# meyer-lab/cmtf-pls

Hardware: AMD Instinct MI355X
Metric: nipals_iters_per_sec (higher is better)
Workload: dtype f32

## Files before the change

cmtf_pls_amd/_lib.py:

```python
from __future__ import annotations

import ctypes
import os
from ctypes import c_char_p, c_double, c_int, c_int64, c_size_t, c_uint32, c_uint64, c_void_p

_HERE = os.path.dirname(os.path.abspath(__file__))
LIB_PATH = os.environ.get("CMTFPLS_LIB") or os.path.join(_HERE, "lib", "libcmtfpls.so")

_P = c_void_p

class XcovBlock(ctypes.Structure):
    _fields_ = [("S", _P), ("S2", _P), ("colcnt", _P), ("n_samples", c_double), ("order", c_int), ("A", c_int), ("B", c_int),
                ("n_squarings", c_int), ("Z", _P), ("wA", _P), ("wB", _P), ("info", _P)]


class KfoldState(ctypes.Structure):
    _fields_ = [("I", c_int), ("A", c_int), ("B", c_int), ("M", c_int), ("K", c_int), ("R", c_int)] + [
        (name, _P) for name in ("fold_of", "S", "mean", "Yk", "Gy", "WA", "WB", "Q", "Wa", "Wb", "T", "Gt", "coef", "Rm", "tm",
                                "Tout", "vec", "n_iter", "status", "part")]


class CvCoupledBlock(ctypes.Structure):
    _fields_ = [("X", _P), ("order", c_int), ("A", c_int), ("B", c_int)]


class LooCoupledBlock(ctypes.Structure):
    _fields_ = [("X", _P), ("colsum", _P), ("order", c_int), ("A", c_int), ("B", c_int)]


SIGNATURES = {
    "cmtfpls_xcov_iterate_blocks_f64": (c_int, [ctypes.POINTER(XcovBlock), c_int, c_int, _P, _P, _P, _P, _P, c_int, _P, c_size_t, _P]),
    "cmtfpls_abi_version": (c_int, []),
    "cmtfpls_last_error": (c_char_p, []),
    "cmtfpls_clear_error": (c_int, []),
    "cmtfpls_status_to_host": (c_int, [_P, _P, c_size_t, _P, _P]),
    "cmtfpls_colstats_workspace_bytes": (c_size_t, [c_int64, c_int64]),
    "cmtfpls_colstats_f32": (c_int, [_P, c_int64, c_int64, _P, _P, _P, c_size_t, _P]),
    "cmtfpls_colstats_f64": (c_int, [_P, c_int64, c_int64, _P, _P, _P, c_size_t, _P]),
    "cmtfpls_sweep_partials": (c_int, []),
    "cmtfpls_center_f32": (c_int, [_P, c_int64, c_int64, _P, _P, _P, _P]),
    "cmtfpls_center_f64": (c_int, [_P, c_int64, c_int64, _P, _P, _P, _P]),
    "cmtfpls_mode0_contract_workspace_bytes": (c_size_t, [c_int64, c_int64]),
# ... 115 lines not shown
                                          _P, _P, c_size_t, _P]),
    "cmtfpls_heldout_resid_f64": (c_int, [_P, c_int64, c_int, c_int, _P, c_int, c_int, _P, _P, _P, c_double, c_uint64, c_uint32, c_uint64,
                                          _P, _P, c_size_t, _P]),
    "cmtfpls_impute_workspace_bytes": (c_size_t, [c_int64, c_int64]),
    "cmtfpls_impute_f32": (c_int, [_P, _P, c_int64, c_int, c_int, _P, c_int, c_int, _P, _P, _P, _P, _P, c_size_t, _P]),
    "cmtfpls_impute_f64": (c_int, [_P, _P, c_int64, c_int, c_int, _P, c_int, c_int, _P, _P, _P, _P, _P, c_size_t, _P]),
    "cmtfpls_loo_fold_workspace_bytes": (c_size_t, [c_int, c_int, c_int, c_int, c_int]),
    "cmtfpls_loo_tpls_f64": (c_int, [_P, _P, _P, _P, c_int, c_int, c_int, c_int, c_int, c_double, c_int, c_int, c_int, _P, _P, _P, c_size_t, _P]),
    "cmtfpls_loo_xcov_fold_workspace_bytes": (c_size_t, [c_int, c_int, c_int, c_int, c_int]),
    "cmtfpls_kfold_xcov_workspace_bytes": (c_size_t, [c_int64, c_int64, c_int, c_int]),
    "cmtfpls_kfold_xcov_f32": (c_int, [_P, c_int64, c_int, c_int, _P, c_int, _P, _P, c_int, _P, _P, _P, _P, _P, c_size_t, _P]),
    "cmtfpls_kfold_xcov_f64": (c_int, [_P, c_int64, c_int, c_int, _P, c_int, _P, _P, c_int, _P, _P, _P, _P, _P, c_size_t, _P]),
    "cmtfpls_kfold_xcov_bf16": (c_int, [_P, c_int64, c_int, c_int, _P, c_int, _P, _P, c_int, _P, _P, _P, _P, _P, c_size_t, _P]),
    "cmtfpls_kfold_xcov_f16": (c_int, [_P, c_int64, c_int, c_int, _P, c_int, _P, _P, c_int, _P, _P, _P, _P, _P, c_size_t, _P]),
    "cmtfpls_kfold_row_tiles": (c_int, [c_int64]),
    "cmtfpls_kfold_part_stride": (c_int, []),
    "cmtfpls_kfold_inner_workspace_bytes": (c_size_t, [c_int, c_int, c_int]),
    "cmtfpls_kfold_inner_f64": (c_int, [ctypes.POINTER(KfoldState), c_int, c_double, c_int, _P, c_size_t, _P]),
    "cmtfpls_kfold_inner_tensor_workspace_bytes": (c_size_t, [c_int, c_int, c_int, c_int]),
    "cmtfpls_kfold_inner_tensor_lds_bytes": (c_size_t, [c_int, c_int, c_int, c_int]),
    "cmtfpls_kfold_inner_tensor_f64": (c_int, [ctypes.POINTER(KfoldState), _P, c_int, c_int, c_int, c_int, c_double, c_int, _P, _P, _P,
                                       c_size_t, _P]),
    "cmtfpls_kfold_epilogue_f64": (c_int, [ctypes.POINTER(KfoldState), c_int, c_int, _P, _P]),
    "cmtfpls_kfold_inner_coupled_workspace_bytes": (c_size_t, [ctypes.POINTER(KfoldState), c_int]),
    "cmtfpls_kfold_inner_coupled_f64": (c_int, [ctypes.POINTER(KfoldState), c_int, c_int, c_double, c_int, _P, c_size_t, _P]),
    "cmtfpls_kfold_inner_coupled_tensor_workspace_bytes": (c_size_t, [ctypes.POINTER(KfoldState), c_int, ctypes.POINTER(c_int)]),
    "cmtfpls_kfold_inner_coupled_tensor_lds_bytes": (c_size_t, [ctypes.POINTER(KfoldState), c_int, ctypes.POINTER(c_int)]),
    "cmtfpls_kfold_inner_coupled_tensor_f64": (c_int, [ctypes.POINTER(KfoldState), c_int, ctypes.POINTER(c_int), _P, c_int, c_int, c_double,
                                                       c_int, _P, _P, _P, c_size_t, _P]),
    "cmtfpls_kfold_combine_scores_f64": (c_int, [_P, c_int, c_int64, _P, _P]),
    "cmtfpls_kfold_wide_xcov_workspace_bytes": (c_size_t, [c_int64, c_int64, c_int, c_int]),
    "cmtfpls_kfold_wide_xcov_f32": (c_int, [_P, c_int64, c_int, c_int, _P, c_int, _P, _P, c_int, _P, _P, _P, _P, _P, c_size_t, _P]),
    "cmtfpls_kfold_wide_xcov_f64": (c_int, [_P, c_int64, c_int, c_int, _P, c_int, _P, _P, c_int, _P, _P, _P, _P, _P, c_size_t, _P]),
    "cmtfpls_kfold_wide_xcov_bf16": (c_int, [_P, c_int64, c_int, c_int, _P, c_int, _P, _P, c_int, _P, _P, _P, _P, _P, c_size_t, _P]),
    "cmtfpls_kfold_wide_xcov_f16": (c_int, [_P, c_int64, c_int, c_int, _P, c_int, _P, _P, c_int, _P, _P, _P, _P, _P, c_size_t, _P]),
    "cmtfpls_kfold_inner_grouped_f64": (c_int, [ctypes.POINTER(KfoldState), _P, c_int, c_int, c_double, c_int, _P, c_size_t, _P]),
    "cmtfpls_kfold_inner_coupled_grouped_f64": (c_int, [ctypes.POINTER(KfoldState), c_int, _P, c_int, c_int, c_double, c_int, _P, c_size_t,
                                                        _P]),
    "cmtfpls_kfold_epilogue_grouped_f64": (c_int, [ctypes.POINTER(KfoldState), _P, c_int, c_int, c_int, _P, _P]),
    "cmtfpls_kfold_epilogue_splits_f64": (c_int, [ctypes.POINTER(KfoldState), c_int, c_int, c_int, _P, _P]),
    "cmtfpls_kfold_weighted_xcov_workspace_bytes": (c_size_t, [c_int64, c_int64, c_int, c_int]),
    "cmtfpls_kfold_weighted_xcov_f32": (c_int, [_P, c_int64, c_int, c_int, _P, c_int, c_int, _P, _P, _P, _P, c_size_t, _P]),
    "cmtfpls_kfold_weighted_xcov_f64": (c_int, [_P, c_int64, c_int, c_int, _P, c_int, c_int, _P, _P, _P, _P, c_size_t, _P]),
    "cmtfpls_kfold_weighted_xcov_bf16": (c_int, [_P, c_int64, c_int, c_int, _P, c_int, c_int, _P, _P, _P, _P, c_size_t, _P]),
    "cmtfpls_kfold_weighted_xcov_f16": (c_int, [_P, c_int64, c_int, c_int, _P, c_int, c_int, _P, _P, _P, _P, c_size_t, _P]),
    "cmtfpls_kfold_epilogue_weighted_f64": (c_int, [ctypes.POINTER(KfoldState), c_int, c_int, _P, _P]),
# ... 78 lines not shown
```

cmtf_pls_amd/backend.py:

```python
from __future__ import annotations

import ctypes
from typing import Optional, Tuple

import torch

from . import _lib
from .storage import HALF_DTYPES, HALF_ENTRIES, SUFFIX, entry_name

_HALF_ENTRIES = tuple(dict.fromkeys(e for group in HALF_ENTRIES.values() for e in group))


def _ptr(t: Optional[torch.Tensor]):
    return None if t is None else t.data_ptr()


def _int_pairs(pairs):
    flat = [int(v) for p in pairs for v in p]
    return (ctypes.c_int * len(flat))(*flat)


def _scratch(nbytes: int, device) -> torch.Tensor:
    return torch.empty(max(int(nbytes), 256), dtype=torch.uint8, device=device)

# ... 304 lines not shown
        keep = (blocks, q_cur, tq, q_new, G, status, wr, arr)
        fn, stream = self.lib.cmtfpls_xcov_iterate_blocks_f64, self._stream
        args = (nb, M, _ptr(q_cur), _ptr(tq), _ptr(q_new), _ptr(G), status[0:1].data_ptr())
        tail = (_ptr(wr), wr.numel())

        def enqueue(n_squarings, first: bool, _keep=keep) -> None:
            for i in range(nb):
                arr[i].n_squarings = int(n_squarings[i])
            rc = fn(arr, *args, 1 if first else 0, *tail, stream())
            if rc:
                _lib.check(rc, "xcov_iterate_blocks")
        return enqueue

    def s_downdate(self, S: torch.Tensor, A: int, B: int, ya: torch.Tensor, wA: torch.Tensor, wB: torch.Tensor,
                   q: torch.Tensor, v: torch.Tensor) -> None:
        assert S.is_contiguous() and S.shape[1] == A * B
        _lib.check(self.lib.cmtfpls_s_downdate_f64(_ptr(S), S.shape[0], A, B, _ptr(ya), _ptr(wA), _ptr(wB), _ptr(q), _ptr(v),
                                                   self._stream()), "s_downdate")

    def kr_axpy(self, v: torch.Tensor, A: int, B: int, WA: torch.Tensor, WB: torch.Tensor, k: int, coef: torch.Tensor) -> torch.Tensor:
        assert WA.is_contiguous() and WB.is_contiguous() and WA.shape[1] == WB.shape[1] and coef.numel() >= k
        _lib.check(self.lib.cmtfpls_kr_axpy_f64(_ptr(v), A, B, _ptr(WA), _ptr(WB), WA.shape[1], int(k), _ptr(coef), self._stream()), "kr_axpy")
        return v

    def axpy_scalar(self, y: torch.Tensor, a: torch.Tensor, x: Optional[torch.Tensor] = None) -> torch.Tensor:
        assert y.is_contiguous() and y.dtype == torch.float64 and a.numel() >= 1 and (x is None or (x.is_contiguous() and x.numel() == y.numel()))
        _lib.check(self.lib.cmtfpls_axpy_scalar_f64(_ptr(y), y.numel(), _ptr(a), _ptr(x), self._stream()), "axpy_scalar")
        return y

    def total(self, v: torch.Tensor) -> torch.Tensor:
        assert v.is_contiguous() and v.dtype == torch.float64
        return self._close_partials(v)

    def quadform(self, G: torch.Tensor, q: torch.Tensor, q_old: torch.Tensor, out: torch.Tensor) -> torch.Tensor:
        _lib.check(self.lib.cmtfpls_quadform_f64(_ptr(G), G.shape[0], _ptr(q), _ptr(q_old), _ptr(out), self._stream()), "quadform")
        return out

    def mttkrp(self, X2: torch.Tensor, A: int, B: int, WA: torch.Tensor, WB: torch.Tensor, out: torch.Tensor,
               mixed: bool = False) -> Optional[torch.Tensor]:
        R = WA.shape[1]
        assert WA.is_contiguous() and WB.is_contiguous() and out.stride(1) == 1
        fn = self._read_fn("mttkrp", X2, mixed)
        if fn is None:
            return None
        rc = fn(_ptr(X2), X2.shape[0], A, B, _ptr(WA), _ptr(WB), R, _ptr(out), out.stride(0), self._stream())
        return self._form(rc, "mttkrp", out)
# ... 608 lines not shown
```

cmtf_pls_amd/csrc/solve.hip:

```cpp
#include "common.hpp"

namespace cmtfpls {

constexpr int kSolveMax = 64;

__global__ __launch_bounds__(kSolveMax) void normal_solve_kernel(const double* __restrict__ G, const double* __restrict__ g, int k,
                                                                double* __restrict__ b, int incb) {
  __shared__ double A[kSolveMax][kSolveMax + 1];
  __shared__ double d[kSolveMax], y[kSolveMax];
  __shared__ int dep[kSolveMax];
  const int i = threadIdx.x;
  if (i < k) {
    const double gii = G[(int64_t)i * k + i];
    d[i] = (gii > 0.0 && isfinite(gii)) ? 1.0 / sqrt(gii) : 0.0;
    dep[i] = 0;
  }
  __syncthreads();
  if (i < k) {
    for (int j = 0; j < k; ++j) A[i][j] = G[(int64_t)i * k + j] * d[i] * d[j];
    y[i] = g[i] * d[i];
  }
  __syncthreads();
  const double tiny = (double)k * 2.220446049250313e-16;
  for (int c = 0; c < k; ++c) {
    const double piv = A[c][c];
    const bool ok = piv > tiny;
    __syncthreads();
    if (ok) {
      const double l = sqrt(piv);
      if (i == c) A[c][c] = l;
      if (i > c && i < k) A[i][c] = A[i][c] / l;
    } else {
      if (i == c) { A[c][c] = 1.0; dep[c] = 1; }
      if (i > c && i < k) A[i][c] = 0.0;
    }
    __syncthreads();
    if (ok && i > c && i < k) {
      const double lic = A[i][c];
      for (int j = c + 1; j <= i; ++j) A[i][j] -= lic * A[j][c];
    }
    __syncthreads();
  }
  if (i == 0) {
    for (int r = 0; r < k; ++r) {
      double s = y[r];
      for (int j = 0; j < r; ++j) s -= A[r][j] * y[j];
      y[r] = dep[r] ? 0.0 : s / A[r][r];
    }
    for (int r = k - 1; r >= 0; --r) {
      double s = y[r];
      for (int j = r + 1; j < k; ++j) s -= A[j][r] * y[j];
      y[r] = dep[r] ? 0.0 : s / A[r][r];
    }
  }
  __syncthreads();
  if (i < k) b[(int64_t)i * incb] = y[i] * d[i];
}

constexpr int kSolveBigMax = 1024;
__global__ __launch_bounds__(256) void normal_solve_big_kernel(const double* __restrict__ G, const double* __restrict__ g, int k,
                                                               double* __restrict__ b, int incb, double* __restrict__ Aw) {
  const int ld = k + 1;
  double* d = Aw + (size_t)k * ld;
  double* y = d + k;
  double* depf = y + k;
  __shared__ double s_piv;
  const int t = threadIdx.x;
  for (int i = t; i < k; i += 256) {
    const double gii = G[(int64_t)i * k + i];
    d[i] = (gii > 0.0 && isfinite(gii)) ? 1.0 / sqrt(gii) : 0.0;
    depf[i] = 0.0;
  }
  __syncthreads();
  for (int i = t; i < k; i += 256) {
    for (int j = 0; j < k; ++j) Aw[(size_t)i * ld + j] = G[(int64_t)i * k + j] * d[i] * d[j];
    y[i] = g[i] * d[i];
  }
  __syncthreads();
  const double tiny = (double)k * 2.220446049250313e-16;
// ... 181 lines not shown
```

cmtf_pls_amd/fitrun.py:

```python
from __future__ import annotations

import math
from typing import Dict, List, Optional

import numpy as np
import torch

from .fitrun_xcov import XcovMixin
from .sparsity import SWITCHED_OFF, resolve_sparsity, validate_sparse_limits
from .state import BlockState, FitState, split_trailing, validate_limits
from .storage import HALF_DTYPES, HALF_ENTRIES, dtype_name, fallback_text, half_route


class FitRun(XcovMixin):

    def __init__(self, eng: NipalsEngine, Xs: List[torch.Tensor], Y: torch.Tensor, n_components: int, coupled: bool,
                 algorithm: str = "direct", owned: Optional[List[bool]] = None, allow_raw: bool = True, sparsity=None):
        be, comm = eng.be, eng.comm
        Xs = list(Xs)
        owned = [True] * len(Xs) if owned is None else list(owned)
        if algorithm not in ("direct", "xcov"):
            raise ValueError("algorithm must be 'direct' or 'xcov'")
        self.algorithm_requested = self.algorithm = algorithm
        self.notes: List[str] = []
# ... 258 lines not shown
            if self.S12[b] is not None:
                self.Yw[:, :self.M].copy_(self.Y)
                torch.mul(self.Y, self.rowscale[b][:, None], out=self.Yw[:, self.M:])
                be.xcov(self.X2[b], self.Yw, True, out=self.S12[b], mixed=self.mixed)
                comm.allreduce(self.S12[b])
                continue
            if b in self._s_prebuilt:
                del self._s_prebuilt[b]
            elif self.raw and self._ssq_with_s and b not in self._ssq0_dev:
                _, ssq = be.xcov_ssq(self.X2[b], self.Y, blk.mean, out=self.S[b])
                self._ssq0_dev[b] = comm.allreduce(ssq)
            else:
                be.xcov(self.X2[b], self.Y, blk.has_miss, out=self.S[b], mixed=self.mixed)
            comm.allreduce(self.S[b])
            if self.raw:
                ysum, _ = be.colstats(self.Y)
                comm.allreduce(ysum)
                be.s_downdate(self.S[b], blk.A, blk.B, self.zM, self.zA[b], self.zB[b], ysum, blk.mean)
            if blk.has_miss:
                torch.mul(self.Y, self.rowscale[b][:, None], out=self.Yw)
                be.xcov(self.X2[b], self.Yw, True, out=self.S2[b], mixed=self.mixed)
                comm.allreduce(self.S2[b])
        self._s_ready = False
        be.gram_tn(self.Y, self.Y, out=self.Gy)
        comm.allreduce(self.Gy)
        self._parity = 0
        self.qc = self.qx[0]
        self.qc.zero_()
        self.qc[0] = 1.0

    def inner_loop(self, a: int, max_iter: int, tol: float, verbose: int = 0) -> None:
        if max_iter > 0 and self._pipeline_ok():
            self._pipelined = True
            self._inner_loop_xcov_pipelined(a, max_iter, tol, verbose)
            return
        for it in range(max_iter):
            du = self.iterate(it)
            if du is not None and du < tol:
                if verbose:
                    print("Comp {}: converged after {} iterations".format(a, it))
                break

    def _sparse_arg(self, b: int):
        if self.sparse is None:
            return None
        return self.sparse[b], (self.sparse_info[b] if len(self.blocks[b].shape) == 3 else None)

    def _sparse_count(self, b: int) -> None:
        if self.sparse is None or len(self.blocks[b].shape) != 3:
            return
        acc, inf = self.sparse_acc[b], self.sparse_info[b]
        acc[0:1].add_(1.0 - inf[0:1])
# ... 431 lines not shown
            rep["x_copy"] = "centred private copy"
        else:
            nowrite = bool(getattr(self, "_nowrite", False))
            one_read = nowrite and bool(getattr(self, "_one_read", False))
            any_miss = any(b.has_miss for b in self.blocks)
            rep["x_copy"] = "none: the caller's uncentred tensor is read in place" if self.raw else "centred private copy"
            rep["raw"] = bool(self.raw)
            rep["x_written"] = not nowrite
            rep["s_carried"] = bool(self._s_carry)
            rep["s_build"] = ("per component (missing values)" if any_miss else "first component only") + \
                             (f", {(self.M + 63) // 64} response tiles of <= 64" if self.M > 64 else "") + \
                             (", [Y, Y * rowscale] in one pass" if any(x is not None for x in self.S12) else "")
            rep["one_read"] = one_read
            rep["stats_with_s"] = bool(getattr(self, "_stats_with_s", False))
            if nowrite:
                rep["x_passes_per_component"] = ("1 read (largest block); 2 reads (other blocks)" if one_read and nb > 1 else
                                                 "1 read" if one_read else "2 reads")
            elif any_miss and nb == 1 and getattr(self, "_deflate_build_ok", True) and self.S12[0] is not None and eng.opt.xcov_deflate_build:
                rep["x_passes_per_component"] = "1 read + 1 read + write (deflation inside the rebuild of S)"
            elif any_miss:
                rep["x_passes_per_component"] = "1 read + write (score + deflation) + S rebuild reads"
            else:
                rep["x_passes_per_component"] = "1 read + 1 read + write"
            rep["pipelined"] = bool(getattr(self, "_pipelined", False))
            if rep["pipelined"]:
                rep["pipeline"] = dict(self.pipeline_stats)
            if not rep["pipelined"] and eng.opt.xcov_pipeline:
                why = ("sparse loadings" if self.sparse is not None else "graph replay requested" if self.use_graphs else "more than 64 responses" if self.M > 64 else
                       "a block of order > 3 or a backend without the single-call iteration")
                self.notes.append("inner loop on S not pipelined: " + why)
            if self.algorithm_requested == "xcov" and not self.raw and eng.opt.xcov_raw and not any_miss and not any("uncentred" in n for n in self.notes):
                self.notes.append("uncentred xcov form declined: " + ("more than 64 components" if self.R > 64 else
                                                                      "f32 matrix precision or a backend without its kernels"))
            if nowrite and eng.opt.xcov_one_read and self.R > 1 and not one_read:
                self.notes.append("one read per component declined: the row does not fit the registers of 1..16 workgroups "
                                  "(rows of 2048..131072 f32 -- 262144 when the last mode divides 4096 -- / 1024..131072 f64 elements, "
                                  "last mode a multiple of 4 / 2)")
        if any(d is not None for d in self.half_storage):
            rep["half_storage"] = {
                "in_place": self.half_fallback is None,
                "fallback": self.half_fallback,
                "reads": [None if d is None or self.half_fallback is not None else self._half_reads_form(b)
                          for b, d in enumerate(self.half_storage)],
            }
        rep["rank1_one_launch_chain"] = bool(getattr(eng.be, "rank1_chain_side", 0)) and any(
            len(blk.shape) == 3 and min(blk.A, blk.B) <= int(getattr(eng.be, "rank1_chain_side", 0)) for blk in self.blocks)
# ... 30 lines not shown
```

cmtf_pls_amd/fitrun_xcov.py:

```python
from __future__ import annotations

import math
from typing import Optional

import torch

from .storage import HALF_DTYPES


class XcovMixin:
    def _score_x0(self, b: int, out: torch.Tensor) -> None:
        be, blk, X2 = self.eng.be, self.blocks[b], self.X2[b]
        if X2.dtype in HALF_DTYPES:
            self.half_reads.setdefault(b, set()).add("mttkrp")
            if be.mttkrp(X2, blk.A, blk.B, self.wA[b].view(-1, 1), self.wB[b].view(-1, 1), out.view(-1, 1)) is None:
                raise RuntimeError("mttkrp refused a shape the 16-bit fit was planned for")
        else:
            be.score(X2, blk.A, blk.B, self.wA[b], self.wB[b], None, out)

    def _contract_x0(self, b: int, v: torch.Tensor, out: torch.Tensor) -> None:
        be, X2 = self.eng.be, self.X2[b]
        if X2.dtype in HALF_DTYPES:
            self.half_reads.setdefault(b, set()).add("xcov")
            if be.xcov(X2, v.view(-1, 1), False, out=out.view(1, -1)) is None:
# ... 236 lines not shown
                if a > 0:
                    be.rowdot(self.T[:, :a], g, self.corr, None)
                    corr = self.corr
                if nb == 2:
                    others = self.Ts[1 - b]
                elif nb > 2:
                    others = self.Ts[[x for x in range(nb) if x != b]].sum(dim=0)
                one_read = be.score_contract(self.X2[b], blk.A, blk.B, self.wA[b], self.wB[b], mw, self.Ts[b], self.ps,
                                             sub_own=corr, add_other=others, alpha=1.0 / nb,
                                             csum=self.csum if self.raw else None) is not None
                if one_read:
                    if self.X2[b].dtype in HALF_DTYPES:
                        self.half_reads.setdefault(b, set()).add("score_contract")
                    continue
                self._one_read = False
            self._score_x0(b, self.Ts[b])
            if mw is not None:
                be.axpy_scalar(self.Ts[b], mw)
            if a > 0:
                be.y_deflate(self.Ts[b].view(I, 1), self.T, a, g, self.one)
        single = self.t.data_ptr() == self.Ts.data_ptr()
        if not single:
            be.scores_mean(self.Ts, self.t)
        if one_read:
            comm.allreduce(self.ps)
            if self.raw:
                be.axpy_scalar(self.ps, comm.allreduce(self.csum), self.blocks[fused_b].mean)
            self.Rm[:, a].copy_(self.ps)
        be.rowdot(self.Y, self.q, self.u, None)
        be.gram_tn(self.t, self.t, out=self.dot_log[a, 0:1])
        for b in range(nb):
            if single:
                self.dot_log[a, 1 + b].copy_(self.dot_log[a, 0])
            else:
                be.gram_tn(self.Ts[b], self.t, out=self.dot_log[a, 1 + b: 2 + b])
        self.T[:, a].copy_(self.t)
        self.U[:, a].copy_(self.u)
        self.Q[:, a].copy_(self.q)
        Ta = self.T[:, :k]
        ya = be.gram_tn(self.Y, self.t).reshape(-1)
        b_dev, ya_g = self._inner_regression(a, extra=ya)
        if k < R and not (one_read and nb == 1):
            be.rowdot(Ta, b_dev, self.yhat.view(-1), None)
        ssqy = be.y_deflate(self.Y, self.T, k, b_dev, self.q)
        if k < R:
            c = be.gram_tn(self._G_last, b_dev).reshape(-1)
            for b, blk in enumerate(self.blocks):
                WA, WB = self.eng._kr_operands(blk, R)
                if one_read and b == fused_b:
                    be.rowdot(self.Rm[:, :k], b_dev, self.vs[b], None)
                else:
                    self._contract_x0(b, self.yhat.view(-1), self.vs[b])
                    comm.allreduce(self.vs[b])
                    if self.raw:
                        be.axpy_scalar(self.vs[b], comm.allreduce(be.total(self.yhat.view(-1))), blk.mean)
                be.kr_axpy(self.vs[b], blk.A, blk.B, WA, WB, k, c)
                be.s_downdate(self.S[b], blk.A, blk.B, ya_g, self.wA[b], self.wB[b], self.q, self.vs[b])
            self._s_ready = True
        self.ssq_log[a, nb].copy_(ssqy.reshape(()))
```

cmtf_pls_amd/options.py:

```python
from __future__ import annotations

from dataclasses import dataclass, replace
from typing import Optional


@dataclass(frozen=True)
class EngineOptions:
    small_fit: bool = True
    small_fit_elements: int = 1 << 15
    xcov_nowrite: bool = True
    xcov_raw: bool = True
    xcov_raw_max_offset: float = 1e4
    project_raw_max_offset: float = 1e4
    xcov_one_read: bool = True
    xcov_pair_build: bool = True
    xcov_ssq_with_s: bool = True
    xcov_stats_with_s: bool = True
    xcov_deflate_build: bool = True
    xcov_pipeline: bool = True
    capture_collectives: bool = False
    project_split_rows: bool = True
    masked_folds: bool = False
    masked_folds_coupled: bool = False
    coupled_permutations: bool = False
    tensor_folds: bool = False
    tensor_folds_coupled: bool = False
    masked_tensor_folds: bool = False
    tensor_resamples_coupled: bool = False
    masked_tensor_folds_coupled: bool = False
    half_folds: bool = False
    half_diagnostics: bool = False
    sparse_tol: float = 1e-10
    sparse_max_sweeps: int = 200

    def but(self, **changes) -> "EngineOptions":
        return replace(self, **changes)

# ... 13 lines not shown
```

include/cmtfpls.h:

```cpp
#ifndef CMTFPLS_H
#define CMTFPLS_H

#include <stddef.h>
#include <stdint.h>

#ifdef __cplusplus
extern "C" {
#endif

#define CMTFPLS_OK 0
#define CMTFPLS_EINVAL 1
#define CMTFPLS_EWORKSPACE 2
#define CMTFPLS_EHIP 3
#define CMTFPLS_EUNSUPPORTED 4

int cmtfpls_abi_version(void);
const char* cmtfpls_last_error(void);
int cmtfpls_clear_error(void);
int cmtfpls_status_to_host(const void* src, void* dst_host, size_t bytes, void* event, void* stream);

size_t cmtfpls_colstats_workspace_bytes(int64_t I, int64_t P);
int cmtfpls_colstats_f32(const float* X, int64_t I, int64_t P, double* colsum, double* colcnt,
                         void* ws, size_t ws_bytes, void* stream);
int cmtfpls_colstats_f64(const double* X, int64_t I, int64_t P, double* colsum, double* colcnt,
// ... 397 lines not shown
int cmtfpls_kfold_inner_coupled_grouped_f64(const cmtfpls_kfold_state* blocks, int nb, const int* model_fold, int groups, int a, double tol,
                                            int max_iter, void* ws, size_t ws_bytes, void* stream);

int cmtfpls_kfold_epilogue_splits_f64(const cmtfpls_kfold_state* st, int splits, int stage, int a, const double* in, void* stream);

size_t cmtfpls_kfold_weighted_xcov_workspace_bytes(int64_t I, int64_t P, int n, int M);
int cmtfpls_kfold_weighted_xcov_f32(const float* X, int64_t I, int A, int B, const double* Y, int n, int M, double* S, double* mean,
                                    double* stats, void* ws, size_t ws_bytes, void* stream);
int cmtfpls_kfold_weighted_xcov_f64(const double* X, int64_t I, int A, int B, const double* Y, int n, int M, double* S, double* mean,
                                    double* stats, void* ws, size_t ws_bytes, void* stream);
int cmtfpls_kfold_weighted_xcov_bf16(const uint16_t* X, int64_t I, int A, int B, const double* Y, int n, int M, double* S, double* mean,
                                     double* stats, void* ws, size_t ws_bytes, void* stream);
int cmtfpls_kfold_weighted_xcov_f16(const uint16_t* X, int64_t I, int A, int B, const double* Y, int n, int M, double* S, double* mean,
                                    double* stats, void* ws, size_t ws_bytes, void* stream);
int cmtfpls_kfold_epilogue_weighted_f64(const cmtfpls_kfold_state* st, int stage, int a, const double* in, void* stream);
size_t cmtfpls_press_rows_workspace_bytes(int n, int64_t I, int R, int M);
int cmtfpls_press_rows_f64(const double* T, const double* coef, const double* Q, const double* nu, const double* Y, const int* eval,
                           int n, int64_t I, int R, int M, double* press, double* pred, void* ws, size_t ws_bytes, void* stream);
size_t cmtfpls_fit_small_workspace_bytes(int I, int A, int B, int M);
int cmtfpls_fit_small_f64(const double* X, const double* Y, int I, int A, int B, int M, int R, double tol, int max_iter,
                          double* T, double* U, double* WA, double* WB, double* Q, double* coef, double* ssq, double* x_mean,
                          double* y_mean, int* n_iter, int* flag, void* ws, size_t ws_bytes, void* stream);

int cmtfpls_add_noise_f32(float* X, int64_t n, double sigma, uint64_t seed, uint64_t offset, double nan_fraction,
                          void* stream);
int cmtfpls_add_noise_f64(double* X, int64_t n, double sigma, uint64_t seed, uint64_t offset, double nan_fraction,
                          void* stream);

int cmtfpls_ceiling_max_blocks(void);
int cmtfpls_ceiling_read(const void* buf, size_t bytes, int64_t row_bytes, int map, float* sink, int blocks, void* stream);
int cmtfpls_ceiling_rmw(void* buf, size_t bytes, int64_t row_bytes, int map, int blocks, void* stream);
int cmtfpls_ceiling_copy(const void* src, void* dst, size_t bytes, int64_t row_bytes, int map, int blocks, void* stream);

#ifdef __cplusplus
}
#endif
#endif
```

Measured before the change: 764.6.

## Fuse per-component NIPALS boundary steps into five tiled device launches

Adds a device entry that does the end-of-component work (score/U store, T'T and T'U reductions, normal-equation solve, Y deflation with Gy rebuild, S downdate, q reset) in five kernels. Before, this was a long sequence of separate small launches and host-driven steps. The fit path now calls it for single order-3 blocks and skips the Gy recompute and q reset afterwards. The intent is to cut launch count and host overhead at component boundaries, at the cost of a large new code path with fixed tiling and shape limits.

Result: no change. 763.9 (-0.1%).

```diff
diff --git a/cmtf_pls_amd/_lib.py b/cmtf_pls_amd/_lib.py
--- a/cmtf_pls_amd/_lib.py
+++ b/cmtf_pls_amd/_lib.py
@@ -18,6 +18,12 @@
     _fields_ = [("I", c_int), ("A", c_int), ("B", c_int), ("M", c_int), ("K", c_int), ("R", c_int)] + [
         (name, _P) for name in ("fold_of", "S", "mean", "Yk", "Gy", "WA", "WB", "Q", "Wa", "Wb", "T", "Gt", "coef", "Rm", "tm",
                                 "Tout", "vec", "n_iter", "status", "part")]
+
+
+class XcovBoundaryArgs(ctypes.Structure):
+    _fields_ = [("I", c_int64)] + [(name, c_int) for name in ("M", "R", "a", "A", "B", "raw")] + [
+        (name, _P) for name in ("t", "Y", "q", "T", "U", "G", "b", "coef", "c", "ya", "dots", "Q", "wA", "wB", "LA", "LB", "q_next",
+                                "Gy", "ssq", "S", "ps", "csum", "mean", "Rm")]
 
 
 class CvCoupledBlock(ctypes.Structure):
@@ -179,6 +185,9 @@
     "cmtfpls_kfold_inner_tensor_f64": (c_int, [ctypes.POINTER(KfoldState), _P, c_int, c_int, c_int, c_int, c_double, c_int, _P, _P, _P,
                                        c_size_t, _P]),
     "cmtfpls_kfold_epilogue_f64": (c_int, [ctypes.POINTER(KfoldState), c_int, c_int, _P, _P]),
+    "cmtfpls_xcov_boundary_tiles": (c_int, []),
+    "cmtfpls_xcov_boundary_workspace_bytes": (c_size_t, [c_int64, c_int, c_int, c_int64]),
+    "cmtfpls_xcov_boundary_f64": (c_int, [ctypes.POINTER(XcovBoundaryArgs), c_int, _P, c_size_t, _P]),
     "cmtfpls_kfold_inner_coupled_workspace_bytes": (c_size_t, [ctypes.POINTER(KfoldState), c_int]),
     "cmtfpls_kfold_inner_coupled_f64": (c_int, [ctypes.POINTER(KfoldState), c_int, c_int, c_double, c_int, _P, c_size_t, _P]),
     "cmtfpls_kfold_inner_coupled_tensor_workspace_bytes": (c_size_t, [ctypes.POINTER(KfoldState), c_int, ctypes.POINTER(c_int)]),
diff --git a/cmtf_pls_amd/backend.py b/cmtf_pls_amd/backend.py
--- a/cmtf_pls_amd/backend.py
+++ b/cmtf_pls_amd/backend.py
@@ -350,6 +350,24 @@
         assert WA.is_contiguous() and WB.is_contiguous() and WA.shape[1] == WB.shape[1] and coef.numel() >= k
         _lib.check(self.lib.cmtfpls_kr_axpy_f64(_ptr(v), A, B, _ptr(WA), _ptr(WB), WA.shape[1], int(k), _ptr(coef), self._stream()), "kr_axpy")
         return v
+
+    def xcov_boundary_args(self, **fields):
+        args = _lib.XcovBoundaryArgs()
+        for name, value in fields.items():
+            self.xcov_boundary_set(args, name, value)
+        return args
+
+    @staticmethod
+    def xcov_boundary_set(args, name: str, value) -> None:
+        if isinstance(value, torch.Tensor):
+            assert value.dtype == torch.float64 and value.is_contiguous(), name
+            value = value.data_ptr()
+        setattr(args, name, value)
+
+    def xcov_boundary(self, args, stage: int = 0) -> Optional[bool]:
+        ws = self._workspace("xcov_boundary", self.lib.cmtfpls_xcov_boundary_workspace_bytes(args.I, args.M, args.R, args.A * args.B))
+        rc = self.lib.cmtfpls_xcov_boundary_f64(ctypes.byref(args), int(stage), _ptr(ws), ws.numel(), self._stream())
+        return self._form(rc, "xcov_boundary")
 
     def axpy_scalar(self, y: torch.Tensor, a: torch.Tensor, x: Optional[torch.Tensor] = None) -> torch.Tensor:
         assert y.is_contiguous() and y.dtype == torch.float64 and a.numel() >= 1 and (x is None or (x.is_contiguous() and x.numel() == y.numel()))
diff --git a/cmtf_pls_amd/csrc/boundary.hip b/cmtf_pls_amd/csrc/boundary.hip
--- /dev/null
+++ b/cmtf_pls_amd/csrc/boundary.hip
@@ -0,0 +1,312 @@
+#include "common.hpp"
+#include "normal_solve.hpp"
+
+namespace cmtfpls {
+
+constexpr int kBndTiles = 256;
+constexpr int kBndMaxM = 64, kBndMaxR = 64;
+constexpr int kBndStage = 4096;
+
+__device__ __forceinline__ void bnd_reduce16(const double (&acc)[16], int n, double (*red)[16], double* out) {
+  const int lane = threadIdx.x & 63, wv = threadIdx.x >> 6;
+#pragma unroll
+  for (int e = 0; e < 16; ++e) {
+    const double w = wave_sum(acc[e]);
+    if (lane == 0) red[wv][e] = w;
+  }
+  __syncthreads();
+  if ((int)threadIdx.x < n) {
+    const int e = threadIdx.x;
+    out[e] = ((red[0][e] + red[1][e]) + red[2][e]) + red[3][e];
+  }
+  __syncthreads();
+}
+
+__global__ __launch_bounds__(256) void boundary_rows_kernel(cmtfpls_xcov_boundary_args p, double* __restrict__ part) {
+  __shared__ double red[4][16];
+  __shared__ double qs[kBndMaxM];
+  const int tid = threadIdx.x;
+  const int M = p.M, R = p.R, a = p.a, k = a + 1;
+  const int64_t I = p.I;
+  for (int m = tid; m < M; m += 256) qs[m] = p.q[m];
+  __syncthreads();
+  const int64_t first = (int64_t)blockIdx.x * 256 + tid, step = (int64_t)kBndTiles * 256;
+  double* out = part + (int64_t)blockIdx.x * (2 * R + M);
+  if (M <= 16) {
+    double acc[16];
+#pragma unroll
+    for (int e = 0; e < 16; ++e) acc[e] = 0.0;
+    for (int64_t i = first; i < I; i += step) {
+      const double ti = p.t[i];
+      const double* yr = p.Y + i * M;
+      double s = 0.0;
+#pragma unroll
+      for (int e = 0; e < 16; ++e)
+        if (e < M) {
+          const double y = yr[e];
+          s = fma(y, qs[e], s);
+          acc[e] = fma(y, ti, acc[e]);
+        }
+      p.U[i * R + a] = s;
+      p.T[i * R + a] = ti;
+    }
+    bnd_reduce16(acc, M, red, out + 2 * R);
+  } else {
+    for (int64_t i = first; i < I; i += step) {
+      const double* yr = p.Y + i * M;
+      double s = 0.0;
+      for (int m = 0; m < M; ++m) s = fma(yr[m], qs[m], s);
+      p.U[i * R + a] = s;
+      p.T[i * R + a] = p.t[i];
+    }
+  }
+  __syncthreads();
+  for (int m0 = 0; m0 < M && M > 16; m0 += 16) {
+    const int mc = (M - m0 < 16) ? M - m0 : 16;
+    double acc[16];
+#pragma unroll
+    for (int e = 0; e < 16; ++e) acc[e] = 0.0;
+    for (int64_t i = first; i < I; i += step) {
+      const double ti = p.t[i];
+      const double* yr = p.Y + i * M + m0;
+#pragma unroll
+      for (int e = 0; e < 16; ++e)
+        if (e < mc) acc[e] = fma(yr[e], ti, acc[e]);
+    }
+    bnd_reduce16(acc, mc, red, out + 2 * R + m0);
+  }
+  for (int j0 = 0; j0 < k; j0 += 16) {
+    const int jc = (k - j0 < 16) ? k - j0 : 16;
+    double at[16], au[16];
+#pragma unroll
+    for (int e = 0; e < 16; ++e) { at[e] = 0.0; au[e] = 0.0; }
+    for (int64_t i = first; i < I; i += step) {
+      const double ti = p.t[i], ui = p.U[i * R + a];
+      const double* tr = p.T + i * R + j0;
+#pragma unroll
+      for (int e = 0; e < 16; ++e)
+        if (e < jc) {
+          const double tv = tr[e];
+          at[e] = fma(tv, ti, at[e]);
+          au[e] = fma(tv, ui, au[e]);
+        }
+    }
+    bnd_reduce16(at, jc, red, out + j0);
+    bnd_reduce16(au, jc, red, out + R + j0);
+  }
+}
+
+__global__ __launch_bounds__(256) void boundary_solve_kernel(cmtfpls_xcov_boundary_args p, const double* __restrict__ part) {
+  __shared__ NormalSolveLds s;
+  __shared__ double tt[kBndMaxR], tu[kBndMaxR], bs[kBndMaxR];
+  const int tid = threadIdx.x;
+  const int M = p.M, R = p.R, a = p.a, k = a + 1, stride = 2 * R + M;
+  const int lane = tid & 63, wv = tid >> 6;
+  for (int o = wv; o < 2 * k + M; o += 4) {
+    const int col = (o < k) ? o : (o < 2 * k) ? R + (o - k) : 2 * R + (o - 2 * k);
+    double v = 0.0;
+    for (int tile = lane; tile < kBndTiles; tile += 64) v += part[(int64_t)tile * stride + col];
+    v = wave_sum(v);
+    if (lane == 0) {
+      if (o < k) tt[o] = v;
+      else if (o < 2 * k) tu[o - k] = v;
+      else p.ya[o - 2 * k] = v;
+    }
+  }
+  __syncthreads();
+  if (tid < k) {
+    p.G[(int64_t)a * R + tid] = tt[tid];
+    p.G[(int64_t)tid * R + a] = tt[tid];
+  }
+  if (tid == 0) { p.dots[0] = tt[a]; p.dots[1] = tt[a]; }
+  __syncthreads();
+  const double bi = normal_solve_block(p.G, R, tu, k, s);
+  if (tid < k) {
+    bs[tid] = bi;
+    p.b[tid] = bi;
+    p.coef[(int64_t)tid * R + a] = bi;
+  }
+  __syncthreads();
+  if (tid < k) {
+    double v = 0.0;
+    for (int j = 0; j < k; ++j) v = fma(p.G[(int64_t)tid * R + j], bs[j], v);
+    p.c[tid] = v;
+  }
+  for (int m = tid; m < M; m += 256) p.Q[(int64_t)m * R + a] = p.q[m];
+  for (int i = tid; i < p.A; i += 256) p.LA[(int64_t)i * R + a] = p.wA[i];
+  for (int i = tid; i < p.B; i += 256) p.LB[(int64_t)i * R + a] = p.wB[i];
+}
+
+__global__ __launch_bounds__(256) void boundary_ydefl_kernel(cmtfpls_xcov_boundary_args p, double* __restrict__ part) {
+  __shared__ double Ys[kBndStage];
+  __shared__ double qs[kBndMaxM], bs[kBndMaxR], red[16];
+  const int tid = threadIdx.x;
+  const int M = p.M, R = p.R, k = p.a + 1, MM = M * M, TR = (kBndStage / M < 256) ? kBndStage / M : 256;
+  for (int m = tid; m < M; m += 256) qs[m] = p.q[m];
+  for (int j = tid; j < k; j += 256) bs[j] = p.b[j];
+  __syncthreads();
+  const int64_t rows_per = (p.I + kBndTiles - 1) / kBndTiles;
+  const int64_t r0 = (int64_t)blockIdx.x * rows_per;
+  const int64_t r1 = (r0 + rows_per < p.I) ? r0 + rows_per : p.I;
+  double ssq = 0.0;
+  double acc[16];
+#pragma unroll
+  for (int e = 0; e < 16; ++e) acc[e] = 0.0;
+  for (int64_t rb = r0; rb < r1; rb += TR) {
+    const int nr = (int)((r1 - rb < TR) ? r1 - rb : TR);
+    if (tid < nr) {
+      const int64_t i = rb + tid;
+      double yh = 0.0;
+      for (int j = 0; j < k; ++j) yh = fma(p.T[i * R + j], bs[j], yh);
+      double* yr = p.Y + i * M;
+      for (int m = 0; m < M; ++m) {
+        const double v = yr[m] - yh * qs[m];
+        yr[m] = v;
+        Ys[tid * M + m] = v;
+        ssq = fma(v, v, ssq);
+      }
+    }
+    __syncthreads();
+#pragma unroll
+    for (int e = 0; e < 16; ++e) {
+      const int o = tid + e * 256;
+      if (o < MM) {
+        const int m1 = o / M, m2 = o % M;
+        double v = acc[e];
+        for (int r = 0; r < nr; ++r) v = fma(Ys[r * M + m1], Ys[r * M + m2], v);
+        acc[e] = v;
+      }
+    }
+    __syncthreads();
+  }
+  double* out = part + (int64_t)blockIdx.x * (MM + 1);
+#pragma unroll
+  for (int e = 0; e < 16; ++e) {
+    const int o = tid + e * 256;
+    if (o < MM) out[o] = acc[e];
+  }
+  const double tot = block_sum(ssq, red);
+  if (tid == 0) out[MM] = tot;
+}
+
+__global__ __launch_bounds__(256) void boundary_close_kernel(cmtfpls_xcov_boundary_args p, const double* __restrict__ part) {
+  const int M = p.M, MM = M * M;
+  const int o = blockIdx.x * 4 + (threadIdx.x >> 6), lane = threadIdx.x & 63;
+  if (o <= MM) {
+    double v = 0.0;
+    for (int tile = lane; tile < kBndTiles; tile += 64) v += part[(int64_t)tile * (MM + 1) + o];
+    v = wave_sum(v);
+    if (lane == 0) {
+      if (o < MM) p.Gy[o] = v;
+      else p.ssq[0] = v;
+    }
+  }
+  if (blockIdx.x == 0 && p.q_next && (int)threadIdx.x < M) p.q_next[threadIdx.x] = threadIdx.x == 0 ? 1.0 : 0.0;
+}
+
+__global__ __launch_bounds__(256) void boundary_downdate_kernel(cmtfpls_xcov_boundary_args p) {
+  __shared__ double bs[kBndMaxR], cs[kBndMaxR], yas[kBndMaxM], qs[kBndMaxM];
+  const int tid = threadIdx.x;
+  const int M = p.M, R = p.R, a = p.a, k = a + 1, B = p.B;
+  for (int j = tid; j < k; j += 256) { bs[j] = p.b[j]; cs[j] = p.c[j]; }
+  for (int m = tid; m < M; m += 256) { yas[m] = p.ya[m]; qs[m] = p.q[m]; }
+  __syncthreads();
+  const int64_t P = (int64_t)p.A * B;
+  const int64_t c = (int64_t)blockIdx.x * 256 + tid;
+  if (c >= P) return;
+  const int64_t ia = c / B, ib = c % B;
+  double r = p.ps[c];
+  if (p.raw) r = fma(-p.csum[0], p.mean[c], r);
+  double* rm = p.Rm + c * R;
+  rm[a] = r;
+  double v = 0.0;
+  for (int j = 0; j < a; ++j) v = fma(rm[j], bs[j], v);
+  v = fma(r, bs[a], v);
+  const double* wa = p.LA + ia * R;
+  const double* wb = p.LB + ib * R;
+  double w2 = 0.0;
+  for (int j = 0; j < k; ++j) w2 = fma(cs[j] * wa[j], wb[j], w2);
+  v -= w2;
+  const double w = p.wA[ia] * p.wB[ib];
+  for (int m = 0; m < M; ++m) {
+    double sv = p.S[(int64_t)m * P + c];
+    sv = fma(-yas[m], w, sv);
+    sv = fma(-qs[m], v, sv);
+    p.S[(int64_t)m * P + c] = sv;
+  }
+}
+
+static size_t bnd_part1(int M, int R) { return (size_t)kBndTiles * (size_t)(2 * R + M); }
+static size_t bnd_part3(int M) { return (size_t)kBndTiles * (size_t)(M * M + 1); }
+
+}
+
+using namespace cmtfpls;
+
+extern "C" {
+
+int cmtfpls_xcov_boundary_tiles(void) { return kBndTiles; }
+
+size_t cmtfpls_xcov_boundary_workspace_bytes(int64_t I, int M, int R, int64_t P) {
+  (void)I;
+  (void)P;
+  if (M <= 0 || R <= 0 || M > kBndMaxM || R > kBndMaxR) return 0;
+  return (bnd_part1(M, R) + bnd_part3(M)) * sizeof(double);
+}
+
+int cmtfpls_xcov_boundary_f64(const cmtfpls_xcov_boundary_args* p, int stage, void* ws, size_t ws_bytes, void* stream) {
+  if (!p || stage < 0 || stage > 5) { set_error("xcov_boundary: bad argument"); return CMTFPLS_EINVAL; }
+  if (p->I <= 0 || p->M <= 0 || p->R <= 0 || p->A <= 0 || p->B <= 0 || p->a < 0 || p->a >= p->R) {
+    set_error("xcov_boundary: bad argument");
+    return CMTFPLS_EINVAL;
+  }
+  if (p->M > kBndMaxM || p->R > kBndMaxR || p->I > ((int64_t)1 << 38) || (int64_t)p->A * p->B > ((int64_t)1 << 38)) {
+    set_error("xcov_boundary: shape outside the device form (M <= 64, R <= 64); use the separate entries");
+    return CMTFPLS_EUNSUPPORTED;
+  }
+  const bool last = p->a + 1 >= p->R;
+  const bool all = stage == 0;
+  const bool s1 = all || stage == 1, s2 = all || stage == 2, s3 = all || stage == 3, s4 = all || stage == 4;
+  const bool s5 = (all && !last) || stage == 5;
+  if (((s1 || s2 || s3 || s5) && !p->q) || (s1 && (!p->t || !p->Y || !p->T || !p->U)) ||
+      (s2 && (!p->G || !p->b || !p->coef || !p->c || !p->ya || !p->dots || !p->Q || !p->wA || !p->wB || !p->LA || !p->LB)) ||
+      (s3 && (!p->Y || !p->T || !p->b)) || (s4 && (!p->Gy || !p->ssq)) ||
+      (s5 && (!p->S || !p->ps || !p->Rm || !p->b || !p->c || !p->ya || !p->wA || !p->wB || !p->LA || !p->LB ||
+              (p->raw && (!p->csum || !p->mean))))) {
+    set_error("xcov_boundary: bad argument");
+    return CMTFPLS_EINVAL;
+  }
+  if (!ws || ws_bytes < cmtfpls_xcov_boundary_workspace_bytes(p->I, p->M, p->R, (int64_t)p->A * p->B)) {
+    set_error("xcov_boundary: workspace too small");
+    return CMTFPLS_EWORKSPACE;
+  }
+  hipStream_t st = (hipStream_t)stream;
+  double* part1 = static_cast<double*>(ws);
+  double* part3 = part1 + bnd_part1(p->M, p->R);
+  const int MM1 = p->M * p->M + 1;
+  const int64_t P = (int64_t)p->A * p->B;
+  int rc = CMTFPLS_OK;
+  if (s1) {
+    hipLaunchKernelGGL(boundary_rows_kernel, dim3(kBndTiles), dim3(256), 0, st, *p, part1);
+    rc = check_launch("xcov_boundary: rows");
+  }
+  if (rc == CMTFPLS_OK && s2) {
+    hipLaunchKernelGGL(boundary_solve_kernel, dim3(1), dim3(256), 0, st, *p, part1);
+    rc = check_launch("xcov_boundary: solve");
+  }
+  if (rc == CMTFPLS_OK && s3) {
+    hipLaunchKernelGGL(boundary_ydefl_kernel, dim3(kBndTiles), dim3(256), 0, st, *p, part3);
+    rc = check_launch("xcov_boundary: ydefl");
+  }
+  if (rc == CMTFPLS_OK && s5) {
+    hipLaunchKernelGGL(boundary_downdate_kernel, dim3((unsigned)((P + 255) / 256)), dim3(256), 0, st, *p);
+    rc = check_launch("xcov_boundary: downdate");
+  }
+  if (rc == CMTFPLS_OK && s4) {
+    hipLaunchKernelGGL(boundary_close_kernel, dim3((unsigned)((MM1 + 3) / 4)), dim3(256), 0, st, *p, part3);
+    rc = check_launch("xcov_boundary: close");
+  }
+  return rc;
+}
+
+}
diff --git a/cmtf_pls_amd/csrc/normal_solve.hpp b/cmtf_pls_amd/csrc/normal_solve.hpp
--- /dev/null
+++ b/cmtf_pls_amd/csrc/normal_solve.hpp
@@ -0,0 +1,63 @@
+#pragma once
+#include "common.hpp"
+
+namespace cmtfpls {
+
+constexpr int kSolveMax = 64;
+
+struct NormalSolveLds {
+  double A[kSolveMax][kSolveMax + 1];
+  double d[kSolveMax], y[kSolveMax];
+  int dep[kSolveMax];
+};
+
+__device__ __forceinline__ double normal_solve_block(const double* G, int ldg, const double* g, int k, NormalSolveLds& s) {
+  const int i = threadIdx.x;
+  if (i < k) {
+    const double gii = G[(int64_t)i * ldg + i];
+    s.d[i] = (gii > 0.0 && isfinite(gii)) ? 1.0 / sqrt(gii) : 0.0;
+    s.dep[i] = 0;
+  }
+  __syncthreads();
+  if (i < k) {
+    for (int j = 0; j < k; ++j) s.A[i][j] = G[(int64_t)i * ldg + j] * s.d[i] * s.d[j];
+    s.y[i] = g[i] * s.d[i];
+  }
+  __syncthreads();
+  const double tiny = (double)k * 2.220446049250313e-16;
+  for (int c = 0; c < k; ++c) {
+    const double piv = s.A[c][c];
+    const bool ok = piv > tiny;
+    __syncthreads();
+    if (ok) {
+      const double l = sqrt(piv);
+      if (i == c) s.A[c][c] = l;
+      if (i > c && i < k) s.A[i][c] = s.A[i][c] / l;
+    } else {
+      if (i == c) { s.A[c][c] = 1.0; s.dep[c] = 1; }
+      if (i > c && i < k) s.A[i][c] = 0.0;
+    }
+    __syncthreads();
+    if (ok && i > c && i < k) {
+      const double lic = s.A[i][c];
+      for (int j = c + 1; j <= i; ++j) s.A[i][j] -= lic * s.A[j][c];
+    }
+    __syncthreads();
+  }
+  if (i == 0) {
+    for (int r = 0; r < k; ++r) {
+      double v = s.y[r];
+      for (int j = 0; j < r; ++j) v -= s.A[r][j] * s.y[j];
+      s.y[r] = s.dep[r] ? 0.0 : v / s.A[r][r];
+    }
+    for (int r = k - 1; r >= 0; --r) {
+      double v = s.y[r];
+      for (int j = r + 1; j < k; ++j) v -= s.A[j][r] * s.y[j];
+      s.y[r] = s.dep[r] ? 0.0 : v / s.A[r][r];
+    }
+  }
+  __syncthreads();
+  return i < k ? s.y[i] * s.d[i] : 0.0;
+}
+
+}
diff --git a/cmtf_pls_amd/csrc/solve.hip b/cmtf_pls_amd/csrc/solve.hip
--- a/cmtf_pls_amd/csrc/solve.hip
+++ b/cmtf_pls_amd/csrc/solve.hip
@@ -1,60 +1,13 @@
 #include "common.hpp"
+#include "normal_solve.hpp"
 
 namespace cmtfpls {
-
-constexpr int kSolveMax = 64;
 
 __global__ __launch_bounds__(kSolveMax) void normal_solve_kernel(const double* __restrict__ G, const double* __restrict__ g, int k,
                                                                 double* __restrict__ b, int incb) {
-  __shared__ double A[kSolveMax][kSolveMax + 1];
-  __shared__ double d[kSolveMax], y[kSolveMax];
-  __shared__ int dep[kSolveMax];
-  const int i = threadIdx.x;
-  if (i < k) {
-    const double gii = G[(int64_t)i * k + i];
-    d[i] = (gii > 0.0 && isfinite(gii)) ? 1.0 / sqrt(gii) : 0.0;
-    dep[i] = 0;
-  }
-  __syncthreads();
-  if (i < k) {
-    for (int j = 0; j < k; ++j) A[i][j] = G[(int64_t)i * k + j] * d[i] * d[j];
-    y[i] = g[i] * d[i];
-  }
-  __syncthreads();
-  const double tiny = (double)k * 2.220446049250313e-16;
-  for (int c = 0; c < k; ++c) {
-    const double piv = A[c][c];
-    const bool ok = piv > tiny;
-    __syncthreads();
-    if (ok) {
-      const double l = sqrt(piv);
-      if (i == c) A[c][c] = l;
-      if (i > c && i < k) A[i][c] = A[i][c] / l;
-    } else {
-      if (i == c) { A[c][c] = 1.0; dep[c] = 1; }
-      if (i > c && i < k) A[i][c] = 0.0;
-    }
-    __syncthreads();
-    if (ok && i > c && i < k) {
-      const double lic = A[i][c];
-      for (int j = c + 1; j <= i; ++j) A[i][j] -= lic * A[j][c];
-    }
-    __syncthreads();
-  }
-  if (i == 0) {
-    for (int r = 0; r < k; ++r) {
-      double s = y[r];
-      for (int j = 0; j < r; ++j) s -= A[r][j] * y[j];
-      y[r] = dep[r] ? 0.0 : s / A[r][r];
-    }
-    for (int r = k - 1; r >= 0; --r) {
-      double s = y[r];
-      for (int j = r + 1; j < k; ++j) s -= A[j][r] * y[j];
-      y[r] = dep[r] ? 0.0 : s / A[r][r];
-    }
-  }
-  __syncthreads();
-  if (i < k) b[(int64_t)i * incb] = y[i] * d[i];
+  __shared__ NormalSolveLds s;
+  const double bi = normal_solve_block(G, k, g, k, s);
+  if ((int)threadIdx.x < k) b[(int64_t)threadIdx.x * incb] = bi;
 }
 
 constexpr int kSolveBigMax = 1024;
diff --git a/cmtf_pls_amd/fitrun.py b/cmtf_pls_amd/fitrun.py
--- a/cmtf_pls_amd/fitrun.py
+++ b/cmtf_pls_amd/fitrun.py
@@ -304,12 +304,16 @@
                 be.xcov(self.X2[b], self.Yw, True, out=self.S2[b], mixed=self.mixed)
                 comm.allreduce(self.S2[b])
         self._s_ready = False
-        be.gram_tn(self.Y, self.Y, out=self.Gy)
-        comm.allreduce(self.Gy)
+        if not getattr(self, "_gy_ready", False):
+            be.gram_tn(self.Y, self.Y, out=self.Gy)
+            comm.allreduce(self.Gy)
+        self._gy_ready = False
         self._parity = 0
         self.qc = self.qx[0]
-        self.qc.zero_()
-        self.qc[0] = 1.0
+        if not getattr(self, "_q_ready", False):
+            self.qc.zero_()
+            self.qc[0] = 1.0
+        self._q_ready = False
 
     def inner_loop(self, a: int, max_iter: int, tol: float, verbose: int = 0) -> None:
         if max_iter > 0 and self._pipeline_ok():
@@ -787,6 +791,11 @@
                 rep["x_passes_per_component"] = "1 read + write (score + deflation) + S rebuild reads"
             else:
                 rep["x_passes_per_component"] = "1 read + 1 read + write"
+            if nowrite:
+                bnd = getattr(self, "_boundary", None) or {"live": False, "why": "no component was finished", "components": 0}
+                rep["boundary"] = ("tiled: 5 launches per component (cmtfpls_xcov_boundary_f64)" if bnd["live"] and bnd["components"]
+                                   else "launch per step")
+                rep["boundary_declined"] = None if bnd["live"] else bnd["why"]
             rep["pipelined"] = bool(getattr(self, "_pipelined", False))
             if rep["pipelined"]:
                 rep["pipeline"] = dict(self.pipeline_stats)
diff --git a/cmtf_pls_amd/fitrun_xcov.py b/cmtf_pls_amd/fitrun_xcov.py
--- a/cmtf_pls_amd/fitrun_xcov.py
+++ b/cmtf_pls_amd/fitrun_xcov.py
@@ -282,6 +282,8 @@
         single = self.t.data_ptr() == self.Ts.data_ptr()
         if not single:
             be.scores_mean(self.Ts, self.t)
+        if self._boundary_tiled(a, one_read):
+            return
         if one_read:
             comm.allreduce(self.ps)
             if self.raw:
@@ -318,3 +320,54 @@
                 be.s_downdate(self.S[b], blk.A, blk.B, ya_g, self.wA[b], self.wB[b], self.q, self.vs[b])
             self._s_ready = True
         self.ssq_log[a, nb].copy_(ssqy.reshape(()))
+
+    def _boundary_declined(self, a: int, one_read: bool) -> Optional[str]:
+        eng, be = self.eng, self.eng.be
+        if not eng.opt.xcov_boundary:
+            return "switched off (EngineOptions.xcov_boundary)"
+        if not hasattr(be, "xcov_boundary"):
+            return "a backend without the entry"
+        if len(self.blocks) != 1 or len(self.blocks[0].shape) != 3:
+            return "not one block of order 3"
+        if eng.comm.sharded:
+            return "a sharded fit"
+        if self.M > 64 or self.R > 64:
+            return "more than 64 responses or components"
+        if not (one_read or a + 1 == self.R):
+            return "the one-read score pass declined the shape"
+        if a > 0 and not self._boundary["live"]:
+            return self._boundary["why"]
+        if not all(v.is_contiguous() and v.dtype == torch.float64 for v in (self.Y, self.t, self.T, self.U, self.Q, self.q, self.S[0])):
+            return "a buffer that is not contiguous float64"
+        return None
+
+    def _boundary_tiled(self, a: int, one_read: bool) -> bool:
+        be = self.eng.be
+        st = getattr(self, "_boundary", None)
+        if st is None:
+            st = self._boundary = {"live": True, "why": None, "components": 0, "args": None}
+        why = self._boundary_declined(a, one_read)
+        if why is None:
+            blk, R = self.blocks[0], self.R
+            last = a + 1 == R
+            args = st["args"]
+            if args is None:
+                st["bufs"] = dict(G=be.zeros(R, R), c=be.empty(R), ya=be.empty(self.M))
+                args = st["args"] = be.xcov_boundary_args(
+                    I=self.I, M=self.M, R=R, A=blk.A, B=blk.B, raw=int(bool(self.raw)), t=self.t, Y=self.Y, T=self.T, U=self.U,
+                    b=self.b_dev, coef=self.coef_dev, Q=self.Q, wA=self.wA[0], wB=self.wB[0], LA=blk.loadings[0], LB=blk.loadings[1],
+                    Gy=self.Gy, S=self.S[0], ps=getattr(self, "ps", None), csum=getattr(self, "csum", None),
+                    mean=blk.mean if self.raw else None, Rm=getattr(self, "Rm", None), **st["bufs"])
+            for name, value in (("a", a), ("q", self.q), ("q_next", None if last else self.qx[0]), ("dots", self.dot_log[a]),
+                                ("ssq", self.ssq_log[a, 1:2])):
+                be.xcov_boundary_set(args, name, value)
+            if be.xcov_boundary(args) is None:
+                why = "the entry declined the shape"
+        if why is not None:
+            st["live"], st["why"] = False, why
+            return False
+        st["components"] += 1
+        self._s_ready = not last
+        self._gy_ready = True
+        self._q_ready = not last
+        return True
diff --git a/cmtf_pls_amd/options.py b/cmtf_pls_amd/options.py
--- a/cmtf_pls_amd/options.py
+++ b/cmtf_pls_amd/options.py
@@ -13,6 +13,7 @@
     xcov_raw_max_offset: float = 1e4
     project_raw_max_offset: float = 1e4
     xcov_one_read: bool = True
+    xcov_boundary: bool = True
     xcov_pair_build: bool = True
     xcov_ssq_with_s: bool = True
     xcov_stats_with_s: bool = True
diff --git a/include/cmtfpls.h b/include/cmtfpls.h
--- a/include/cmtfpls.h
+++ b/include/cmtfpls.h
@@ -443,6 +443,38 @@
                           double* T, double* U, double* WA, double* WB, double* Q, double* coef, double* ssq, double* x_mean,
                           double* y_mean, int* n_iter, int* flag, void* ws, size_t ws_bytes, void* stream);
 
+typedef struct {
+  int64_t I;
+  int M, R, a, A, B, raw;
+  const double* t;
+  double* Y;
+  const double* q;
+  double* T;
+  double* U;
+  double* G;
+  double* b;
+  double* coef;
+  double* c;
+  double* ya;
+  double* dots;
+  double* Q;
+  const double* wA;
+  const double* wB;
+  double* LA;
+  double* LB;
+  double* q_next;
+  double* Gy;
+  double* ssq;
+  double* S;
+  const double* ps;
+  const double* csum;
+  const double* mean;
+  double* Rm;
+} cmtfpls_xcov_boundary_args;
+int cmtfpls_xcov_boundary_tiles(void);
+size_t cmtfpls_xcov_boundary_workspace_bytes(int64_t I, int M, int R, int64_t P);
+int cmtfpls_xcov_boundary_f64(const cmtfpls_xcov_boundary_args* p, int stage, void* ws, size_t ws_bytes, void* stream);
+
 int cmtfpls_add_noise_f32(float* X, int64_t n, double sigma, uint64_t seed, uint64_t offset, double nan_fraction,
                           void* stream);
 int cmtfpls_add_noise_f64(double* X, int64_t n, double sigma, uint64_t seed, uint64_t offset, double nan_fraction,
```
